# orhosko/tiny-ntt

Hardware: AMD Instinct MI355X
Metric: negacyclic poly-mults/sec (n=4096, 60-bit q), bit-exact vs cg_ntt.py (higher is better)
Workload: dtype u64; 1 GPU; n=4096, q=2^60-2^14+1 (60-bit), global batch 65536 = 65536 rows on this GPU, LCG-seeded rows resident in HBM (BASELINE configs[2]); n=4096, q=1152921504606830593, rows_per_gpu=65536, global_batch=65536, variant=fused, kernel=polymul_fused_kernel, lazy_reduction=True, lib_build_id=33db21926526ecac, parallelism=batch-sharded x1, no data-path collective

## Files before the change

tiny_ntt_amd/csrc/fused_core.h:

```cpp
#pragma once
#include <type_traits>
#include "modarith.h"

#ifndef TN_ABL_UNIFORM_TW
#define TN_ABL_UNIFORM_TW 0
#endif

namespace tn {

template <int B, int E_, typename F> struct StaticFor {
  TN_HD static void run(F& f) { f(std::integral_constant<int, B>()); StaticFor<B + 1, E_, F>::run(f); }
};
template <int E_, typename F> struct StaticFor<E_, E_, F> { TN_HD static void run(F&) {} };
template <int B, int E_, typename F> TN_HD void static_for(F&& f) { StaticFor<B, E_, F>::run(f); }

#ifndef TN_FUSED_LPT10
#define TN_FUSED_LPT10 3
#endif
#ifndef TN_FUSED_LPT12
#define TN_FUSED_LPT12 3
#endif
constexpr int fused_lpt(int logn) {
  return logn == 8 ? 2 : logn == 9 ? 3 : logn == 10 ? TN_FUSED_LPT10 : logn == 11 ? 3 : logn == 12 ? TN_FUSED_LPT12 : logn == 13 ? 3 : 0;
}

template <typename E> struct Arith {
  E q;
  u64 mu;
  int k;
  u32 fold_c;
  SplitK sk;
  u64 qmul[17];
  typename TwOf<E>::type one;
  typename TwOf<E>::type ninv;
  typename TwOf<E>::type fninv;
  typename TwOf<E>::type fninv_w1;
  typename TwOf<E>::type bninv;
  typename TwOf<E>::type bninv_w1;
};

template <typename E, int LOGN_, int LPT_> struct FusedCfg {
  static constexpr int LOGN = LOGN_, LPT = LPT_;
  static constexpr int N = 1 << LOGN, R = 1 << LPT, THREADS = N >> LPT;
  static constexpr int PHASES = (LOGN + LPT - 1) / LPT;
  static constexpr int pos(int p) { return (LOGN - (p + 1) * LPT) < 0 ? 0 : (LOGN - (p + 1) * LPT); }
  static constexpr int stage_begin(int p) { return p * LPT; }
  static constexpr int stage_end(int p) { return ((p + 1) * LPT) < LOGN ? ((p + 1) * LPT) : LOGN; }
  static constexpr int ex_pad(int e) { return pos(e + 1) > 0 ? (1 << pos(e + 1)) : 1; }
  static constexpr int ex_sh(int e) { return pos(e + 1) > 0 ? pos(e + 1) + LPT : LPT; }
  static constexpr int lay_span(int e, int cnt) { return cnt + ex_pad(e) * (cnt >> ex_sh(e)); }
  static constexpr int WB = (LOGN - LPT > 6) ? (LOGN - LPT - 6) : 0;
  static constexpr int WSH = LOGN - WB;
  static constexpr int tau_bit_to_j(int p, int t) { return t < pos(p) ? t : t + LPT; }
  static constexpr bool ex_wave_local(int e) {
    for (int t = 6; t < LOGN - LPT; ++t)
      if (tau_bit_to_j(e, t) != t + LPT || tau_bit_to_j(e + 1, t) != t + LPT) return false;
    return true;
  }
  static constexpr int region_elems() {
    int m = 1 << WSH;
    for (int e = 0; e + 1 < PHASES; ++e)
      if (ex_wave_local(e) && lay_span(e, 1 << WSH) > m) m = lay_span(e, 1 << WSH);
    return m;
  }
  static constexpr int lds_elems() {
    int m = region_elems() << WB;
    for (int e = 0; e + 1 < PHASES; ++e)
      if (!ex_wave_local(e) && lay_span(e, N) > m) m = lay_span(e, N);
    return m;
  }
  TN_HD static constexpr u32 jidx(int p, u32 tau, u32 r) {
    return ((tau >> pos(p)) << (pos(p) + LPT)) | (r << pos(p)) | (tau & ((1u << pos(p)) - 1u));
  }
  TN_HD static constexpr u32 ex_addr(int e, u32 j) {
    if (WB > 0 && ex_wave_local(e))
      return (j >> WSH) * (u32)region_elems() + (j & ((1u << WSH) - 1u)) + (u32)ex_pad(e) * ((j & ((1u << WSH) - 1u)) >> ex_sh(e));
    return j + (u32)ex_pad(e) * (j >> ex_sh(e));
  }
  TN_HD static constexpr u32 ex_base(int e, int p, u32 tau) { return ex_addr(e, jidx(p, tau, 0)); }
  TN_HD static constexpr u32 ex_off(int e, int p, u32 r) { return ex_addr(e, jidx(p, 0, r)); }
  enum { TW_UNIFORM = 0, TW_WAVE = 1, TW_LDS = 2, TW_REGS = 3, TW_VEC = 4 };
  static constexpr int LDS_TW_MAX_STAGE = 9;
  static constexpr int tw_src(int p) {
    return pos(p) >= LOGN - LPT ? TW_UNIFORM
         : (pos(p) >= 6 ? TW_WAVE : (pos(p) > 0 ? (stage_end(p) <= LDS_TW_MAX_STAGE ? TW_LDS : TW_VEC) : TW_REGS));
  }
  static constexpr int lds_tw_lo() {
    for (int p = 0; p < PHASES; ++p) if (tw_src(p) == TW_LDS) return 1 << stage_begin(p);
    return 0;
  }
  static constexpr int lds_tw_hi() {
    int h = 0;
    for (int p = 0; p < PHASES; ++p) if (tw_src(p) == TW_LDS) h = 1 << stage_end(p);
    return h;
  }
  static constexpr int lds_tw_count() { return lds_tw_hi() - lds_tw_lo(); }
  static constexpr int pre_count(int s) { return R >> ((LOGN - 1 - s) - pos(PHASES - 1) + 1); }
  static constexpr int pre_off(int s) {
    int o = 0;
    for (int i = stage_begin(PHASES - 1); i < s; ++i) o += pre_count(i);
    return o;
  }
  static constexpr int NPRE = (tw_src(PHASES - 1) == TW_REGS) ? pre_off(LOGN) : 1;
  TN_HD static u32 nat_addr(u32 k) { return k ^ ((k >> 5) & 15u); }
  TN_HD static u32 thi(int p, u32 tau) {
    if (pos(p) >= LOGN - LPT) return 0u;
    if (pos(p) >= 6) return wave_uniform(tau >> pos(p));
    return tau >> pos(p);
  }
};

template <typename E> struct LazyTraits;
template <> struct LazyTraits<u64> { static constexpr int LIMIT = 16, TMUL = 4, PW = 2; };
template <> struct LazyTraits<u32> { static constexpr int LIMIT = 64, TMUL = 2, PW = 4; };

template <typename E, bool LAZY, bool CIN = false> struct Policy {
  typedef typename TwOf<E>::type Tw;
  static constexpr bool lazy = LAZY;
  static constexpr bool canonical_inputs = CIN && LAZY && sizeof(E) == 8;
  static constexpr bool split = LAZY && sizeof(E) == 8;
  static constexpr int LIMIT = LazyTraits<E>::LIMIT, TMUL = LazyTraits<E>::TMUL, PW = LazyTraits<E>::PW;

  TN_HD static E load(E x, const Arith<E>& ar) {
    if (canonical_inputs) return x;
    if (LAZY) return fold(x, ar.k, ar.fold_c);
    return mul_tw(x, ar.one, ar.q);
  }
  TN_HD static E canon(E x, const Arith<E>& ar) {
    if (LAZY) { x = fold(x, ar.k, ar.fold_c); return csub(x, ar.q); }
    return x;
  }
  template <int K> TN_HD static void ct(E& u, E& v, Tw w, const Arith<E>& ar) {
    if constexpr (split) {
      const u64 x = mul_sp_acc(u, v, w, ar.sk);
      v = ((u << 1) + ar.qmul[K]) - x;
      u = x;
    } else if constexpr (LAZY) {
      const E t = mul_tw_lazy(v, w, ar.q);
      v = u + ((E)K * ar.q - t);
      u = u + t;
    } else {
      E t = mul_tw(v, w, ar.q);
      E s = u + t;
      v = u >= t ? u - t : u + (ar.q - t);
      u = csub(s, ar.q);
    }
  }
  template <int BND> TN_HD static void gs(E& u, E& v, Tw w, const Arith<E>& ar) {
    if constexpr (split) {
      const E d = (u + ar.qmul[BND]) - v;
      u = u + v;
      v = mul_sp(d, w, ar.sk);
    } else if constexpr (LAZY) {
      const E d = u + ((E)BND * ar.q - v);
      u = u + v;
      v = mul_tw_lazy(d, w, ar.q);
    } else {
      E d = u >= v ? u - v : u + (ar.q - v);
      u = csub(u + v, ar.q);
      v = mul_tw(d, w, ar.q);
    }
  }
  template <int BND> TN_HD static void gs_last(E& u, E& v, const Arith<E>& ar) {
    E d;
    if constexpr (split) d = (u + ar.qmul[BND]) - v;
    else d = LAZY ? (E)(u + ((E)BND * ar.q - v)) : (u >= v ? (E)(u - v) : (E)(u + (ar.q - v)));
    E s = u + v;
    u = mul_tw_canon(s, ar.fninv, ar);
    v = mul_tw_canon(d, ar.fninv_w1, ar);
  }
  TN_HD static E mul_tw_canon(E a, Tw w, const Arith<E>& ar) {
    if constexpr (split) return csub(fold(mul_sp(a, w, ar.sk), ar.k, ar.fold_c), ar.q);
    else return mul_tw(a, w, ar.q);
  }
};

template <typename P, int LOGN> struct Sched {
  static constexpr int fwd_in(int s) {
    int b = 2;
    for (int i = 0; i < s; ++i) { if (b + P::TMUL > P::LIMIT) b = 2; b += P::TMUL; }
    return b;
  }
  static constexpr bool fwd_fold(int s) { return P::lazy && fwd_in(s) + P::TMUL > P::LIMIT; }
  static constexpr int fwd_out() {
    int b = 2;
    for (int i = 0; i < LOGN; ++i) { if (b + P::TMUL > P::LIMIT) b = 2; b += P::TMUL; }
    return b;
  }
  static constexpr int inv_in(int g) {
    int b = P::lazy ? P::PW : 1;
    for (int i = 0; i < g; ++i) { if (2 * b > P::LIMIT) b = 2; b = (2 * b > P::TMUL) ? 2 * b : P::TMUL; }
    return b;
  }
  static constexpr bool inv_fold(int g) { return P::lazy && 2 * inv_in(g) > P::LIMIT; }
  static constexpr int inv_bnd(int g) { return inv_fold(g) ? 2 : inv_in(g); }
};

template <typename Cfg, bool CIN = false, bool BC = false> struct SplitSched {
  static constexpr int LOGN = Cfg::LOGN, R = Cfg::R;
  static constexpr int FEND = BC ? LOGN - 1 : LOGN;
  static constexpr long U = 4096, CAP = 16 * U;
  static constexpr long FOLDED = U + 1;
  static constexpr long PW_OUT = 2 * U;
  static constexpr long PW_IN = 14 * (U - 1);
  static constexpr long tmax(long bv) { return 4 * U + (bv + 7) / 8 + 2; }
  static constexpr long BC_AMAX = CAP - 8;
  static constexpr int kq(long b) { return (int)((b + U - 2) / (U - 1)); }
  static constexpr int kf(long t) { return kq(t) <= 6 ? 6 : kq(t); }
  static constexpr int ki(long b) { return (kq(b) + 3) / 4 * 4; }
  static constexpr int phase_of(int s) { return s / Cfg::LPT; }
  static constexpr int bpos_of(int s) { return (LOGN - 1 - s) - Cfg::pos(phase_of(s)); }
  struct Data {
    bool ffold[LOGN][R] = {};
    unsigned char fk[LOGN][R] = {};
    long fout = 0;
    bool pw_fold_b = false;
    bool bcfold[R] = {};
    bool ifold[LOGN][R] = {};
    unsigned char ik[LOGN][R] = {};
  };
  static constexpr Data build() {
    Data d;
    long b[R] = {};
    for (int r = 0; r < R; ++r) b[r] = CIN ? U : (r < R / 2 ? FOLDED : CAP);
    for (int s = 0; s < FEND; ++s) {
      if (s > 0 && phase_of(s) != phase_of(s - 1)) {
        long m = 0;
        for (int r = 0; r < R; ++r) m = b[r] > m ? b[r] : m;
        for (int r = 0; r < R; ++r) b[r] = m;
      }
// ... 255 lines not shown
```

tiny_ntt_amd/csrc/kernels.hip:

```cpp
#include <hip/hip_runtime.h>
#include "plan.h"
#include "dev_addr.h"

#ifndef TN_ABL_NO_BARRIER
#define TN_ABL_NO_BARRIER 0
#endif
#ifndef TN_ABL_ROWMASK
#define TN_ABL_ROWMASK 0
#endif
#ifndef TN_ABL_NO_GLOBAL
#define TN_ABL_NO_GLOBAL 0
#endif
#ifndef TN_STORE_AT_TOP
#define TN_STORE_AT_TOP 1
#endif
#ifndef TN_NT_STREAM
#define TN_NT_STREAM 1
#endif
#ifndef TN_FUSED_MIN_WAVES
#define TN_FUSED_MIN_WAVES 4
#endif
#ifndef TN_POLYMUL60_WAVES
#define TN_POLYMUL60_WAVES 6
#endif

#ifndef TN_NTTF_PIN_LOGN
#define TN_NTTF_PIN_LOGN 99
#endif
#ifndef TN_VEC_PREFETCH
#define TN_VEC_PREFETCH 1
#endif
#ifndef TN_FUSED_CIN
#define TN_FUSED_CIN 0
#endif
#ifndef TN_SADDR
#define TN_SADDR 1
#endif
#ifndef TN_KARG_ARITH
#define TN_KARG_ARITH 1
#endif
#ifndef TN_RESIDENT_TW
#define TN_RESIDENT_TW 1
#endif
#ifndef TN_SHARE_MID_TW
#define TN_SHARE_MID_TW 1
#endif
#ifndef TN_SHARE_LAST_TW
#define TN_SHARE_LAST_TW 1
#endif
#ifdef TN_MARKS
#define TN_MARK(n) asm volatile("; TNMARK " n)
#else
#define TN_MARK(n)
#endif
namespace tn {

#ifndef TN_SHUFFLE_LAST
#define TN_SHUFFLE_LAST 0
#endif
template <int DIST> __device__ __forceinline__ u32 lane_xor(u32 v) {
  if constexpr (DIST == 1) return (u32)__builtin_amdgcn_update_dpp(0, (int)v, 0xB1, 0xf, 0xf, false);
  else if constexpr (DIST == 2) return (u32)__builtin_amdgcn_update_dpp(0, (int)v, 0x4E, 0xf, 0xf, false);
  else {
    int r = __builtin_amdgcn_update_dpp(0, (int)v, 0x104, 0xf, 0x5, false);
    return (u32)__builtin_amdgcn_update_dpp(r, (int)v, 0x114, 0xf, 0xA, false);
  }
}
template <typename E>
__device__ __forceinline__ void transpose8_lanes(E (&x)[8], u32 lane) {
  static_for<0, 3>([&](auto b_) {
    constexpr int b = decltype(b_)::value, m = 1 << b;
    const bool hi = (lane >> b) & 1u;
    static_for<0, 8>([&](auto r_) {
      constexpr int r0 = decltype(r_)::value;
      if constexpr (!(r0 & m)) {
        constexpr int r1 = r0 | m;
        const E send = hi ? x[r0] : x[r1];
        E recv;
        if constexpr (sizeof(E) == 8) recv = ((u64)lane_xor<m>((u32)(send >> 32)) << 32) | lane_xor<m>((u32)send);
        else recv = lane_xor<m>((u32)send);
        x[r0] = hi ? recv : x[r0];
        x[r1] = hi ? x[r1] : recv;
      }
    });
  });
}

template <typename E, typename Cfg, int EX, int FROM, int TO>
__device__ __forceinline__ void exchange(E (&x)[Cfg::R], u32 tau, E* lds) {
  if constexpr (TN_SHUFFLE_LAST && Cfg::LPT == 3 && EX == Cfg::PHASES - 2 && Cfg::pos(EX + 1) == 0 && Cfg::pos(EX) == Cfg::LPT) {
    transpose8_lanes<E>(x, tau);
  } else if constexpr (Cfg::ex_wave_local(EX)) {
    __builtin_amdgcn_wave_barrier();
    ex_store<E, Cfg, EX, FROM>(x, tau, lds);
    __builtin_amdgcn_wave_barrier();
    ex_load<E, Cfg, EX, TO>(x, tau, lds);
    __builtin_amdgcn_wave_barrier();
  } else {
#if TN_ABL_NO_BARRIER
    __builtin_amdgcn_wave_barrier();
    ex_store<E, Cfg, EX, FROM>(x, tau, lds);
    __builtin_amdgcn_wave_barrier();
    ex_load<E, Cfg, EX, TO>(x, tau, lds);
    __builtin_amdgcn_wave_barrier();
#else
    __syncthreads();
    ex_store<E, Cfg, EX, FROM>(x, tau, lds);
    __syncthreads();
    ex_load<E, Cfg, EX, TO>(x, tau, lds);
    __syncthreads();
#endif
  }
}

template <typename E>
__device__ __forceinline__ const Arith<E>& kernarg_arith(u32 zero) {
  typedef const __attribute__((address_space(4))) char* KP;
  return *(const Arith<E>*)((KP)__builtin_amdgcn_kernarg_segment_ptr() + zero);
}

template <typename E, typename Cfg, typename Pol, int P0, int P1, bool KARG = false, int PRE_END = Cfg::LOGN, bool BC = false>
__device__ __forceinline__ void forward_range(E (&x)[Cfg::R], u32 tau, const TwRefs<E>& tw_in, const Arith<E>& ar_in, E* lds, bool fetch_pre,
                                              u32 tau_g) {
  typename TwOf<E>::type vec[Cfg::R];
  static_for<P0, P1>([&](auto p_) {
    constexpr int p = decltype(p_)::value;
    constexpr bool FULL = Cfg::stage_end(p) - Cfg::stage_begin(p) == Cfg::LPT;
    TN_MARK("fwd_phase");
    TwRefs<E> tw = tw_in;
    if constexpr (KARG) tw.zero = opaque_zero();
    if constexpr (TN_VEC_PREFETCH && Cfg::tw_src(p) == Cfg::TW_VEC && FULL && p > P0) tw.mid = vec;
    const Arith<E>& ar = KARG ? kernarg_arith<E>(tw.zero) : ar_in;
    fwd_phase<E, Cfg, Pol, p, BC>(x, tau, tw, ar);
    TN_MARK("fwd_other");
    if constexpr (p == Cfg::PHASES - 2) {
      if (fetch_pre) {
        sched_fence();
        tw_prefetch_stages<E, Cfg, Cfg::stage_begin(Cfg::PHASES - 1), PRE_END>(tw.pre, tau_g, tw.glob);
        sched_fence();
      }
    }
    if constexpr (p + 1 < P1) {
      constexpr int pn = p + 1 < Cfg::PHASES ? p + 1 : p;
      if constexpr (TN_VEC_PREFETCH && Cfg::tw_src(pn) == Cfg::TW_VEC && Cfg::stage_end(pn) - Cfg::stage_begin(pn) == Cfg::LPT) {
        sched_fence();
        tw_fetch_vec<E, Cfg, pn>(vec, tau_g, tw.glob);
        sched_fence();
      }
    }
    if constexpr (p + 1 < Cfg::PHASES) exchange<E, Cfg, p, p, p + 1>(x, tau, lds);
  });
}
template <typename E, typename Cfg, typename Pol>
__device__ __forceinline__ void forward_all(E (&x)[Cfg::R], u32 tau, const typename TwOf<E>::type* __restrict__ glob,
                                            const typename TwOf<E>::type* lds_tw, const Arith<E>& ar, E* lds, u32 zero = 0) {
  typename TwOf<E>::type pre[Cfg::NPRE];
  const TwRefs<E> tw = {glob, lds_tw, pre, nullptr, zero};
  forward_range<E, Cfg, Pol, 0, Cfg::PHASES>(x, tau, tw, ar, lds, true, tau);
}

template <typename E, typename Cfg, typename Pol, bool KARG = false, bool BC = false, typename F>
__device__ __forceinline__ void inverse_all(E (&x)[Cfg::R], u32 tau, const TwRefs<E>& tw_in, const Arith<E>& ar_in, E* lds,
                                            F&& after_first) {
  typename TwOf<E>::type vec[Cfg::R];
  static_for<0, Cfg::PHASES>([&](auto i_) {
    constexpr int p = Cfg::PHASES - 1 - decltype(i_)::value;
    constexpr bool FULL = Cfg::stage_end(p) - Cfg::stage_begin(p) == Cfg::LPT;
    TN_MARK("inv_phase");
    TwRefs<E> tw = tw_in;
    if constexpr (KARG) tw.zero = opaque_zero();
    if constexpr (TN_VEC_PREFETCH && Cfg::tw_src(p) == Cfg::TW_VEC && FULL && p < Cfg::PHASES - 1) tw.mid = vec;
    const Arith<E>& ar = KARG ? kernarg_arith<E>(tw.zero) : ar_in;
    inv_phase<E, Cfg, Pol, p, BC>(x, tau, tw, ar);
    TN_MARK("inv_other");
    if constexpr (p > 0) {
      constexpr int pn = p > 0 ? p - 1 : 0;
      if constexpr (TN_VEC_PREFETCH && Cfg::tw_src(pn) == Cfg::TW_VEC && Cfg::stage_end(pn) - Cfg::stage_begin(pn) == Cfg::LPT) {
        sched_fence();
        tw_fetch_vec<E, Cfg, pn>(vec, tau, tw.glob);
        sched_fence();
      }
    }
    if constexpr (p == Cfg::PHASES - 1) { sched_fence(); after_first(); sched_fence(); }
    if constexpr (p > 0) exchange<E, Cfg, p - 1, p, p - 1>(x, tau, lds);
  });
}

template <typename E> struct alignas(2 * sizeof(E)) PairOf { E lo, hi; };

#ifdef TN_FUSED_STAMPS
__device__ unsigned long long tn_fused_stamps[4 * 4096];
#endif

template <typename E, typename Cfg>
__device__ __forceinline__ E ld_operand(const E* __restrict__ p, u32 row, u32 tau, int r) {
#if TN_ABL_NO_GLOBAL
  return (E)(tau * 2654435761u + 7 * r + row);
#else
#if TN_ABL_ROWMASK
  row &= TN_ABL_ROWMASK;
#endif
#if TN_NT_STREAM
  const TN_GLOBAL_AS E* rp = uniform_ptr(p + ((size_t)row << Cfg::LOGN) + Cfg::jidx(0, 0, r));
  return __builtin_nontemporal_load(rp + (Cfg::jidx(0, tau, 0) & (u32)(Cfg::N - 1)));
#else
  return p[((size_t)row << Cfg::LOGN) + Cfg::jidx(0, tau, r)];
#endif
#endif
}

template <typename E, typename Cfg>
__device__ __forceinline__ void st_result(E* __restrict__ c, u32 row, u32 tau, const E (&x)[Cfg::R]) {
#if TN_ABL_ROWMASK
  row &= TN_ABL_ROWMASK;
#endif
  const size_t off = (size_t)row << Cfg::LOGN;
#pragma unroll
  for (int r = 0; r < Cfg::R; ++r) {
#if TN_NT_STREAM
    __builtin_nontemporal_store(x[r], uniform_ptr(c + off + Cfg::jidx(0, 0, r)) + (Cfg::jidx(0, tau, 0) & (u32)(Cfg::N - 1)));
#else
    c[off + Cfg::jidx(0, tau, r)] = x[r];
#endif
  }
}

template <typename E, int LOGN, int LPT, bool LAZY>
constexpr int polymul_waves() {
  return LPT >= 4 ? 2 : (sizeof(E) == 8 && LOGN == 12 && LAZY) ? TN_POLYMUL60_WAVES : TN_FUSED_MIN_WAVES;
}

template <typename E, int LOGN, int LPT, bool LAZY, bool CIN = false, bool BC = false>
__global__ void __launch_bounds__((1 << (LOGN - LPT)), (polymul_waves<E, LOGN, LPT, LAZY>()))
polymul_fused_kernel(const Arith<E> ar, const typename TwOf<E>::type* __restrict__ tab_fwd,
                     const typename TwOf<E>::type* __restrict__ tab_inv, const E* __restrict__ a, const E* __restrict__ b,
                     E* __restrict__ c, u32 batch, u32* sched, u32 chunk) {
  typedef FusedCfg<E, LOGN, LPT> Cfg;
  typedef Policy<E, LAZY, CIN> Pol;
  extern __shared__ __attribute__((aligned(16))) unsigned char tn_smem[];
  E* lds = reinterpret_cast<E*>(tn_smem);
  typedef typename TwOf<E>::type Tw;
  const u32 tau = threadIdx.x;
  Tw* lds_fwd = reinterpret_cast<Tw*>(lds + Cfg::lds_elems());
  Tw* lds_inv = lds_fwd + Cfg::lds_tw_count();
  u32* lds_next = reinterpret_cast<u32*>(lds_inv + Cfg::lds_tw_count());
  for (u32 i = tau; i < (u32)Cfg::lds_tw_count(); i += Cfg::THREADS) {
    lds_fwd[i] = tab_fwd[Cfg::lds_tw_lo() + i];
    lds_inv[i] = tab_inv[Cfg::lds_tw_lo() + i];
  }
  __syncthreads();
  E xa[Cfg::R], xb[Cfg::R];
#ifdef TN_FUSED_STAMPS
  const unsigned long long st_t0 = __builtin_amdgcn_s_memtime(), st_r0 = __builtin_amdgcn_s_memrealtime();
#endif
  u32 row = blockIdx.x * chunk;
  u32 taken = 1;
  u32 chunk_id = blockIdx.x;
  if (row < batch) {
#pragma unroll
    for (int r = 0; r < Cfg::R; ++r) xb[r] = ld_operand<E, Cfg>(a, row, tau, r);
  }
  constexpr int PRE_END = (TN_RESIDENT_TW && polymul_waves<E, LOGN, LPT, LAZY>() <= 4 && Cfg::stage_end(Cfg::PHASES - 1) - Cfg::stage_begin(Cfg::PHASES - 1) >= 2) ? Cfg::LOGN - 1 : Cfg::LOGN;
  Tw prf[Cfg::NPRE];
  tw_prefetch_stages<E, Cfg, PRE_END, Cfg::LOGN>(prf, tau, tab_fwd);
  u32 prev = row;
  bool have_c = false;
#pragma unroll
  for (int r = 0; r < Cfg::R; ++r) xa[r] = 0;
  while (row < batch) {
    const u32 zero = opaque_zero();
    const u32 tl = opaque_copy(tau);
    const bool in_chunk = taken != chunk;
    taken = in_chunk ? taken + 1 : 1;
    chunk_id = in_chunk ? chunk_id : chunk_id + gridDim.x;
    if (tau == 0) *lds_next = in_chunk ? row + 1 : (sched ? gridDim.x + atomicAdd(&sched[0], 1u) : chunk_id) * chunk;
    TN_MARK("loop_top");
    E xn[Cfg::R];
#pragma unroll
    for (int r = 0; r < Cfg::R; ++r) xn[r] = xb[r];
    load_reduce<E, Cfg, Pol>(xn, ar);
    sched_fence();
#if TN_STORE_AT_TOP
    st_result<E, Cfg>(c, prev, tl, xa);
#endif
#pragma unroll
    for (int r = 0; r < Cfg::R; ++r) xb[r] = ld_operand<E, Cfg>(b, row, tl, r);
    sched_fence();
#pragma unroll
    for (int r = 0; r < Cfg::R; ++r) xa[r] = xn[r];
    constexpr bool KARG = TN_KARG_ARITH != 0;
    constexpr bool SHARE = TN_SHARE_LAST_TW && Cfg::PHASES >= 2;
    constexpr int PM = Cfg::PHASES >= 3 ? Cfg::PHASES - 2 : 0;
    constexpr bool SHARE2 = SHARE && TN_SHARE_MID_TW && Cfg::PHASES >= 3 && Cfg::tw_src(PM) == Cfg::TW_LDS &&
                            Cfg::stage_end(PM) - Cfg::stage_begin(PM) == Cfg::LPT;
    const TwRefs<E> twf = {tab_fwd, lds_fwd, prf, nullptr, zero};
    static_assert(!BC || SHARE2, "base case: built for the shared-twiddle schedule only");
    if constexpr (SHARE2) forward_range<E, Cfg, Pol, 0, PM, KARG, Cfg::LOGN, BC>(xa, tau, twf, ar, lds, false, tl);
    else if constexpr (SHARE) forward_range<E, Cfg, Pol, 0, Cfg::PHASES - 1, KARG>(xa, tau, twf, ar, lds, false, tl);
    else forward_all<E, Cfg, Pol>(xa, tau, tab_fwd, lds_fwd, ar, lds, zero);
    __syncthreads();
    const u32 next = wave_uniform(*lds_next);
    load_reduce<E, Cfg, Pol>(xb, ar);
    if constexpr (SHARE2) {
      forward_range<E, Cfg, Pol, 0, PM, KARG, Cfg::LOGN, BC>(xb, tau, twf, ar, lds, false, tl);
      Tw mid[Cfg::R];
      tw_fetch_mid<E, Cfg, PM>(mid, tau, lds_fwd);
      const TwRefs<E> twm = {tab_fwd, lds_fwd, prf, mid, zero};
      forward_range<E, Cfg, Pol, PM, PM + 1, KARG, Cfg::LOGN, BC>(xa, tau, twm, ar, lds, false, tl);
      forward_range<E, Cfg, Pol, PM, PM + 1, KARG, PRE_END, BC>(xb, tau, twm, ar, lds, true, tl);
      forward_range<E, Cfg, Pol, PM + 1, Cfg::PHASES, KARG, Cfg::LOGN, BC>(xb, tau, twf, ar, lds, false, tl);
      forward_range<E, Cfg, Pol, PM + 1, Cfg::PHASES, KARG, Cfg::LOGN, BC>(xa, tau, twf, ar, lds, false, tl);
    } else if constexpr (SHARE) {
      forward_range<E, Cfg, Pol, 0, Cfg::PHASES - 1, KARG, PRE_END>(xb, tau, twf, ar, lds, true, tl);
      forward_range<E, Cfg, Pol, Cfg::PHASES - 1, Cfg::PHASES, KARG>(xb, tau, twf, ar, lds, false, tl);
      forward_range<E, Cfg, Pol, Cfg::PHASES - 1, Cfg::PHASES, KARG>(xa, tau, twf, ar, lds, false, tl);
    } else {
      forward_all<E, Cfg, Pol>(xb, tau, tab_fwd, lds_fwd, ar, lds, zero);
    }
    Tw pre[Cfg::NPRE];
    if constexpr (BC) {
      TN_MARK("basecase");
      basecase<Cfg, Pol>(xa, xb, prf + Cfg::pre_off(Cfg::LOGN - 1), ar);
      sched_fence();
      tw_prefetch_stages<E, Cfg, Cfg::stage_begin(Cfg::PHASES - 1), Cfg::LOGN - 1>(pre, tl, tab_inv);
    } else {
      tw_prefetch<E, Cfg>(pre, tl, tab_inv);
      TN_MARK("pointwise");
      pointwise<E, Cfg, Pol>(xa, xb, ar);
    }
    TN_MARK("after_pointwise");
    const TwRefs<E> twi = {tab_inv, lds_inv, pre, nullptr, zero};
    inverse_all<E, Cfg, Pol, KARG, BC>(xa, tau, twi, ar, lds, [&]() {
      const u32 nrow = next < batch ? next : row;
#pragma unroll
      for (int r = 0; r < Cfg::R; ++r) xb[r] = ld_operand<E, Cfg>(a, nrow, tl, r);
    });
#if TN_STORE_AT_TOP
    prev = row;
    have_c = true;
#else
    st_result<E, Cfg>(c, row, tau, xa);
#endif
    row = next;
  }
  if (have_c) st_result<E, Cfg>(c, prev, tau, xa);
#ifdef TN_FUSED_STAMPS
  if (tau == 0 && blockIdx.x < 4096) {
    tn_fused_stamps[4 * blockIdx.x + 0] = st_t0; tn_fused_stamps[4 * blockIdx.x + 1] = st_r0;
    tn_fused_stamps[4 * blockIdx.x + 2] = __builtin_amdgcn_s_memtime(); tn_fused_stamps[4 * blockIdx.x + 3] = __builtin_amdgcn_s_memrealtime();
  }
#endif
  if (sched && tau == 0 && atomicAdd(&sched[1], 1u) == gridDim.x - 1) { sched[0] = 0; sched[1] = 0; }
}

template <typename E, int LOGN, int LPT, bool LAZY, int MODE>
__global__ void __launch_bounds__((1 << (LOGN - LPT)), (LPT >= 4 ? 2 : TN_FUSED_MIN_WAVES))
ntt_fused_kernel(const Arith<E> ar, const typename TwOf<E>::type* __restrict__ tab, const E* __restrict__ in, E* __restrict__ out, u32 batch,
                 u32* sched, u32 chunk) {
  typedef FusedCfg<E, LOGN, LPT> Cfg;
  typedef Policy<E, LAZY> Pol;
  typedef typename TwOf<E>::type Tw;
  extern __shared__ __attribute__((aligned(16))) unsigned char tn_smem[];
  E* lds = reinterpret_cast<E*>(tn_smem);
  const u32 tau = threadIdx.x;
  E* nat = lds + Cfg::lds_elems();
  Tw* lds_tab = reinterpret_cast<Tw*>(nat + Cfg::N);
  u32* lds_next = reinterpret_cast<u32*>(lds_tab + Cfg::lds_tw_count());
  for (u32 i = tau; i < (u32)Cfg::lds_tw_count(); i += Cfg::THREADS) lds_tab[i] = tab[Cfg::lds_tw_lo() + i];
  u32 left = chunk - 1, chunk_id = blockIdx.x;
  auto take_next = [&](u32 cur, u32 slot) {
    if (left) { --left; lds_next[slot] = cur + 1; }
    else {
      chunk_id = sched ? gridDim.x + atomicAdd(&sched[0], 1u) : chunk_id + gridDim.x;
      left = chunk - 1;
      lds_next[slot] = chunk_id * chunk;
    }
  };
  if (tau == 0) take_next(blockIdx.x * chunk, 1u);
  __syncthreads();
  u32 next = wave_uniform(lds_next[1]);
  constexpr int LAST = Cfg::PHASES - 1;
  E xn[Cfg::R];
  u32 row = blockIdx.x * chunk;
  if (row < batch) {
#pragma unroll
    for (int r = 0; r < Cfg::R; ++r) xn[r] = ld_operand<E, Cfg>(in, row, tau, r);
  }
  for (u32 it = 0; row < batch; ++it) {
    if (tau == 0) take_next(next, it & 1u);
    constexpr bool PIN = LOGN >= TN_NTTF_PIN_LOGN;
    const u32 zero = PIN ? opaque_zero() : 0u;
    const u32 tl = PIN ? opaque_copy(tau) : tau;
    constexpr bool KARG = PIN && TN_KARG_ARITH != 0;
    E x[Cfg::R];
#pragma unroll
    for (int r = 0; r < Cfg::R; ++r) x[r] = xn[r];
    sched_fence();
    if (MODE != FNTT_CYCLIC_INV && next < batch) {
#pragma unroll
      for (int r = 0; r < Cfg::R; ++r) xn[r] = ld_operand<E, Cfg>(in, next, tl, r);
    }
    sched_fence();
    if (MODE == FNTT_CYCLIC_INV) {
#pragma unroll
      for (int r = 0; r < Cfg::R; ++r) x[r] = Pol::load(x[r], ar);
#pragma unroll
      for (int r = 0; r < Cfg::R; ++r) nat[Cfg::nat_addr(Cfg::jidx(0, tau, r))] = x[r];
      __syncthreads();
#pragma unroll
      for (int r = 0; r < Cfg::R; ++r) x[r] = nat[Cfg::nat_addr(bitrev(Cfg::jidx(LAST, tau, r), LOGN))];
      Tw pre[Cfg::NPRE];
      tw_prefetch<E, Cfg>(pre, tl, tab);
      const TwRefs<E> tw = {tab, lds_tab, pre, nullptr, zero};
      inverse_all<E, Cfg, Pol, KARG>(x, tau, tw, ar, lds, [&]() {
        if (next < batch) {
#pragma unroll
          for (int r = 0; r < Cfg::R; ++r) xn[r] = ld_operand<E, Cfg>(in, next, tl, r);
        }
      });
      st_result<E, Cfg>(out, row, tl, x);
    } else {
#pragma unroll
      for (int r = 0; r < Cfg::R / 2; ++r) x[r] = Pol::load(x[r], ar);
      if (!LAZY) {
#pragma unroll
        for (int r = Cfg::R / 2; r < Cfg::R; ++r) x[r] = Pol::load(x[r], ar);
      }
      {
        Tw pre[Cfg::NPRE];
        const TwRefs<E> tw = {tab, lds_tab, pre, nullptr, zero};
        forward_range<E, Cfg, Pol, 0, Cfg::PHASES, KARG>(x, tau, tw, ar, lds, true, tl);
      }
#pragma unroll
      for (int r = 0; r < Cfg::R; ++r)
        nat[Cfg::nat_addr(bitrev(Cfg::jidx(LAST, tau, r), LOGN))] = LAZY ? Pol::canon(x[r], ar) : x[r];
      __syncthreads();
#pragma unroll
      for (int r = 0; r < Cfg::R; ++r) x[r] = nat[Cfg::nat_addr(Cfg::jidx(0, tau, r))];
      st_result<E, Cfg>(out, row, tl, x);
    }
    if (Cfg::THREADS <= 64) __syncthreads();
    row = next;
    next = wave_uniform(lds_next[it & 1u]);
  }
  if (sched && tau == 0 && atomicAdd(&sched[1], 1u) == gridDim.x - 1) { sched[0] = 0; sched[1] = 0; }
}

template <typename E, int LOGN, int LPT, bool LAZY>
static hipError_t launch_nttf_t(const tn_plan* p, int mode, const void* in, void* out, size_t batch, hipStream_t s) {
  typedef FusedCfg<E, LOGN, LPT> Cfg;
  typedef typename TwOf<E>::type Tw;
  const size_t lds_bytes = (size_t)(Cfg::lds_elems() + Cfg::N) * sizeof(E) + (size_t)Cfg::lds_tw_count() * sizeof(Tw) + 16;
  const PlanView<E> pv = make_view<E>(p);
  auto kern = ntt_fused_kernel<E, LOGN, LPT, LAZY, FNTT_TWIST_FWD>;
  if (mode == FNTT_CYCLIC_FWD) kern = ntt_fused_kernel<E, LOGN, LPT, LAZY, FNTT_CYCLIC_FWD>;
  else if (mode != FNTT_TWIST_FWD) kern = ntt_fused_kernel<E, LOGN, LPT, LAZY, FNTT_CYCLIC_INV>;
  const FusedNttSetup<E> su = fused_ntt_setup(pv.ar, mode);
  return launch_persistent(p, s, (const void*)kern, Cfg::THREADS, lds_bytes, Cfg::N * sizeof(E), batch, FUSED_ROWS, [&](u32 grid, u32* sched, u32 chunk) {
    const Tw* tab = fused_table(pv, su.tab);
    const E* in_ = (const E*)in; E* out_ = (E*)out; u32 b32 = (u32)batch;
    Arith<E> ar = su.ar;
    void* args[] = {&ar, &tab, &in_, &out_, &b32, &sched, &chunk};
    return hipLaunchKernel((const void*)kern, dim3(grid), dim3(Cfg::THREADS), args, lds_bytes, s);
  });
}

template <typename E, bool LAZY>
static hipError_t launch_nttf_e(const tn_plan* p, int mode, const void* in, void* out, size_t batch, hipStream_t s) {
#ifdef TN_ONLY_MAIN
  return hipErrorInvalidValue;
#else
  switch (p->logn) {
    case 8: return launch_nttf_t<E, 8, fused_lpt(8), LAZY>(p, mode, in, out, batch, s);
    case 9: return launch_nttf_t<E, 9, fused_lpt(9), LAZY>(p, mode, in, out, batch, s);
    case 10: return launch_nttf_t<E, 10, fused_lpt(10), LAZY>(p, mode, in, out, batch, s);
    case 11: return launch_nttf_t<E, 11, fused_lpt(11), LAZY>(p, mode, in, out, batch, s);
    case 12: return launch_nttf_t<E, 12, fused_lpt(12), LAZY>(p, mode, in, out, batch, s);
    case 13: return launch_nttf_t<E, 13, fused_lpt(13), LAZY>(p, mode, in, out, batch, s);
    default: return hipErrorInvalidValue;
  }
#endif
}

hipError_t launch_ntt_fused(const tn_plan* p, int mode, const void* in, void* out, size_t batch, hipStream_t s) {
  if (batch == 0) return hipSuccess;
  if (p->elem_bytes == 8)
    return p->lazy ? launch_nttf_e<u64, true>(p, mode, in, out, batch, s) : launch_nttf_e<u64, false>(p, mode, in, out, batch, s);
  return p->lazy ? launch_nttf_e<u32, true>(p, mode, in, out, batch, s) : launch_nttf_e<u32, false>(p, mode, in, out, batch, s);
}

bool fused_supported(u32 logn, int) { return fused_lpt((int)logn) != 0; }

template <typename E, int LOGN, int LPT, bool LAZY>
static hipError_t launch_fused_t(const tn_plan* p, const void* a, const void* b, void* c, size_t batch, hipStream_t s, bool cyclic) {
  typedef FusedCfg<E, LOGN, LPT> Cfg;
  const size_t lds_bytes = (size_t)Cfg::lds_elems() * sizeof(E) +
                           (size_t)2 * Cfg::lds_tw_count() * sizeof(typename TwOf<E>::type) + 16;
  constexpr bool HAS_CIN = TN_FUSED_CIN && sizeof(E) == 8 && LOGN == 12 && LAZY;
  constexpr bool HAS_BC = fused_has_bc<E, LOGN, LPT, LAZY>();
  const bool use_cin = HAS_CIN && p->canonical_inputs && !cyclic;
  const bool use_bc = HAS_BC && p->bc_ok && !use_cin;
  auto kern = polymul_fused_kernel<E, LOGN, LPT, LAZY>;
// ... 211 lines not shown
```

tiny_ntt_amd/csrc/launch_plan.h:

```cpp
#pragma once
#include <stddef.h>
#include "fused_core.h"

#ifndef TN_DYNAMIC_ROWS
#define TN_DYNAMIC_ROWS 1
#endif
#ifndef TN_SCHED_CHUNK_BYTES
#define TN_SCHED_CHUNK_BYTES 32768
#endif
#ifndef TN_CG_DYNAMIC_ROWS
#define TN_CG_DYNAMIC_ROWS 1
#endif
#ifndef TN_CG_DYNAMIC_MIN
#define TN_CG_DYNAMIC_MIN 8
#endif
#ifndef TN_CG_CHUNK_BYTES
#define TN_CG_CHUNK_BYTES 32768
#endif

namespace tn {

enum FusedNttMode { FNTT_TWIST_FWD = 0, FNTT_CYCLIC_FWD = 1, FNTT_CYCLIC_INV = 2 };

enum FusedTable { FT_PSI_BRV, FT_PSI_INV_BRV, FT_CYC_BRV, FT_CYC_INV_BRV, FT_PSI_BC, FT_CYC_BC };

constexpr int FUSED_BC_LOGN = 12;
template <typename E, int LOGN, int LPT, bool LAZY> constexpr bool fused_has_bc() {
  return sizeof(E) == 8 && LOGN == FUSED_BC_LOGN && LPT == 3 && LAZY;
}

template <typename E> struct FusedProductSetup { bool bc; Arith<E> ar; FusedTable fwd, inv; };
template <typename E> inline FusedProductSetup<E> fused_product_setup(const Arith<E>& ar, bool bc, bool cyclic) {
  FusedProductSetup<E> s = {bc, ar, cyclic ? FT_CYC_BRV : FT_PSI_BRV, cyclic ? FT_CYC_INV_BRV : FT_PSI_INV_BRV};
  if (bc) { s.ar.fninv = ar.bninv; s.ar.fninv_w1 = ar.bninv_w1; s.fwd = cyclic ? FT_CYC_BC : FT_PSI_BC; }
  if (cyclic) s.ar.fninv_w1 = s.ar.fninv;
  return s;
}

template <typename E> struct FusedNttSetup { Arith<E> ar; FusedTable tab; };
template <typename E> inline FusedNttSetup<E> fused_ntt_setup(const Arith<E>& ar, int mode) {
  FusedNttSetup<E> s = {ar, mode == FNTT_TWIST_FWD ? FT_PSI_BRV : mode == FNTT_CYCLIC_FWD ? FT_CYC_BRV : FT_CYC_INV_BRV};
  if (mode == FNTT_CYCLIC_INV) s.ar.fninv_w1 = s.ar.fninv;
  return s;
}

struct RowPolicy { size_t chunk_bytes, min_chunks; bool enabled, single_rows_without_slot; };
constexpr RowPolicy FUSED_ROWS = {TN_SCHED_CHUNK_BYTES, 4, TN_DYNAMIC_ROWS != 0, false};
constexpr RowPolicy CG_ROWS = {TN_CG_CHUNK_BYTES, TN_CG_DYNAMIC_MIN, TN_CG_DYNAMIC_ROWS != 0, true};

struct RowPlan { u32 chunk; bool dynamic; };
inline RowPlan plan_rows(size_t row_bytes, size_t batch, size_t resident, const RowPolicy& pol) {
  size_t want = pol.chunk_bytes / row_bytes;
  if (want < 1) want = 1;
  if (pol.enabled && batch >= pol.min_chunks * resident * want) return {(u32)want, true};
  return {1u, false};
}

}
```

Baseline: 30.55 million poly-mults/s.

## Drop redundant workgroup barriers around cross-wave LDS exchanges in fused polymul

Makes the leading and trailing __syncthreads around each cross-wave LDS transpose configurable. In the base-case path it replaces them with wave barriers wherever a constexpr ownership analysis shows each wave only touches its own LDS region on that side. It also removes the mid-row barrier that published the next row index, reading it later instead. This cuts workgroup-wide synchronisation stalls per row, at the risk of LDS races if the ownership reasoning is wrong. Optional region-timing instrumentation is added but compiled out by default.

```diff
diff --git a/tiny_ntt_amd/csrc/fused_core.h b/tiny_ntt_amd/csrc/fused_core.h
--- a/tiny_ntt_amd/csrc/fused_core.h
+++ b/tiny_ntt_amd/csrc/fused_core.h
@@ -76,6 +76,12 @@
     if (WB > 0 && ex_wave_local(e))
       return (j >> WSH) * (u32)region_elems() + (j & ((1u << WSH) - 1u)) + (u32)ex_pad(e) * ((j & ((1u << WSH) - 1u)) >> ex_sh(e));
     return j + (u32)ex_pad(e) * (j >> ex_sh(e));
+  }
+  static constexpr bool ex_side_wave_own(int e, int p) {
+    for (u32 tau = 0; tau < (u32)THREADS; ++tau)
+      for (u32 r = 0; r < (u32)R; ++r)
+        if (ex_addr(e, jidx(p, tau, r)) / (u32)region_elems() != (tau >> 6)) return false;
+    return true;
   }
   TN_HD static constexpr u32 ex_base(int e, int p, u32 tau) { return ex_addr(e, jidx(p, tau, 0)); }
   TN_HD static constexpr u32 ex_off(int e, int p, u32 r) { return ex_addr(e, jidx(p, 0, r)); }
diff --git a/tiny_ntt_amd/csrc/kernels.hip b/tiny_ntt_amd/csrc/kernels.hip
--- a/tiny_ntt_amd/csrc/kernels.hip
+++ b/tiny_ntt_amd/csrc/kernels.hip
@@ -45,6 +45,9 @@
 #ifndef TN_SHARE_MID_TW
 #define TN_SHARE_MID_TW 1
 #endif
+#ifndef TN_LEAN_BARRIERS
+#define TN_LEAN_BARRIERS 15
+#endif
 #ifndef TN_SHARE_LAST_TW
 #define TN_SHARE_LAST_TW 1
 #endif
@@ -54,6 +57,32 @@
 #define TN_MARK(n)
 #endif
 namespace tn {
+
+#ifdef TN_FUSED_STAMPS
+enum { RGN_A = 0, RGN_B = 16, RGN_INV = 32,
+       RGN_LOOP_TOP = 48, RGN_MID = 49, RGN_B_LOAD = 50, RGN_BASECASE = 51, RGN_AFTER_FIRST = 52, RGN_ROW = 62, RGN_ROWS = 63, RGN_COUNT = 64 };
+__device__ __forceinline__ unsigned long long* rgn_acc() {
+  __shared__ unsigned long long acc[RGN_COUNT];
+  return acc;
+}
+template <int ID, bool END> __device__ __forceinline__ void rgn_stamp() {
+  if constexpr (ID >= 0) {
+    sched_fence();
+    if (threadIdx.x == 0) {
+      const unsigned long long t = __builtin_amdgcn_s_memtime();
+      __hip_atomic_fetch_add(rgn_acc() + ID, END ? t : 0ull - t, __ATOMIC_RELAXED, __HIP_MEMORY_SCOPE_WORKGROUP);
+    }
+    sched_fence();
+  }
+}
+#define TN_RGN_BEGIN(id) rgn_stamp<(id), false>()
+#define TN_RGN_END(id) rgn_stamp<(id), true>()
+#define TN_RGN(base, off) ((base) < 0 ? -1 : (base) + (off))
+#else
+#define TN_RGN_BEGIN(id)
+#define TN_RGN_END(id)
+#define TN_RGN(base, off) (-1)
+#endif
 
 #ifndef TN_SHUFFLE_LAST
 #define TN_SHUFFLE_LAST 0
@@ -86,7 +115,7 @@
   });
 }
 
-template <typename E, typename Cfg, int EX, int FROM, int TO>
+template <typename E, typename Cfg, int EX, int FROM, int TO, int XBAR = XBAR_ALL, int RGW = -1>
 __device__ __forceinline__ void exchange(E (&x)[Cfg::R], u32 tau, E* lds) {
   if constexpr (TN_SHUFFLE_LAST && Cfg::LPT == 3 && EX == Cfg::PHASES - 2 && Cfg::pos(EX + 1) == 0 && Cfg::pos(EX) == Cfg::LPT) {
     transpose8_lanes<E>(x, tau);
@@ -104,11 +133,17 @@
     ex_load<E, Cfg, EX, TO>(x, tau, lds);
     __builtin_amdgcn_wave_barrier();
 #else
+    TN_RGN_BEGIN(RGW);
+    if constexpr (XBAR & XBAR_LEAD) __syncthreads(); else __builtin_amdgcn_wave_barrier();
+    TN_RGN_END(RGW);
+    ex_store<E, Cfg, EX, FROM>(x, tau, lds);
+    TN_RGN_BEGIN(RGW);
     __syncthreads();
-    ex_store<E, Cfg, EX, FROM>(x, tau, lds);
-    __syncthreads();
+    TN_RGN_END(RGW);
     ex_load<E, Cfg, EX, TO>(x, tau, lds);
-    __syncthreads();
+    TN_RGN_BEGIN(RGW);
+    if constexpr (XBAR & XBAR_TRAIL) __syncthreads(); else __builtin_amdgcn_wave_barrier();
+    TN_RGN_END(RGW);
 #endif
   }
 }
@@ -119,7 +154,8 @@
   return *(const Arith<E>*)((KP)__builtin_amdgcn_kernarg_segment_ptr() + zero);
 }
 
-template <typename E, typename Cfg, typename Pol, int P0, int P1, bool KARG = false, int PRE_END = Cfg::LOGN, bool BC = false>
+template <typename E, typename Cfg, typename Pol, int P0, int P1, bool KARG = false, int PRE_END = Cfg::LOGN, bool BC = false, int XBAR = XBAR_ALL,
+          int RG = -1>
 __device__ __forceinline__ void forward_range(E (&x)[Cfg::R], u32 tau, const TwRefs<E>& tw_in, const Arith<E>& ar_in, E* lds, bool fetch_pre,
                                               u32 tau_g) {
   typename TwOf<E>::type vec[Cfg::R];
@@ -127,6 +163,7 @@
     constexpr int p = decltype(p_)::value;
     constexpr bool FULL = Cfg::stage_end(p) - Cfg::stage_begin(p) == Cfg::LPT;
     TN_MARK("fwd_phase");
+    TN_RGN_BEGIN(TN_RGN(RG, 4 * p));
     TwRefs<E> tw = tw_in;
     if constexpr (KARG) tw.zero = opaque_zero();
     if constexpr (TN_VEC_PREFETCH && Cfg::tw_src(p) == Cfg::TW_VEC && FULL && p > P0) tw.mid = vec;
@@ -148,7 +185,12 @@
         sched_fence();
       }
     }
-    if constexpr (p + 1 < Cfg::PHASES) exchange<E, Cfg, p, p, p + 1>(x, tau, lds);
+    TN_RGN_END(TN_RGN(RG, 4 * p));
+    if constexpr (p + 1 < Cfg::PHASES) {
+      TN_RGN_BEGIN(TN_RGN(RG, 4 * p + 1));
+      exchange<E, Cfg, p, p, p + 1, XBAR, TN_RGN(RG, 4 * p + 2)>(x, tau, lds);
+      TN_RGN_END(TN_RGN(RG, 4 * p + 1));
+    }
   });
 }
 template <typename E, typename Cfg, typename Pol>
@@ -159,7 +201,7 @@
   forward_range<E, Cfg, Pol, 0, Cfg::PHASES>(x, tau, tw, ar, lds, true, tau);
 }
 
-template <typename E, typename Cfg, typename Pol, bool KARG = false, bool BC = false, typename F>
+template <typename E, typename Cfg, typename Pol, bool KARG = false, bool BC = false, int XBAR = XBAR_ALL, int RG = -1, typename F>
 __device__ __forceinline__ void inverse_all(E (&x)[Cfg::R], u32 tau, const TwRefs<E>& tw_in, const Arith<E>& ar_in, E* lds,
                                             F&& after_first) {
   typename TwOf<E>::type vec[Cfg::R];
@@ -167,6 +209,7 @@
     constexpr int p = Cfg::PHASES - 1 - decltype(i_)::value;
     constexpr bool FULL = Cfg::stage_end(p) - Cfg::stage_begin(p) == Cfg::LPT;
     TN_MARK("inv_phase");
+    TN_RGN_BEGIN(TN_RGN(RG, 4 * p));
     TwRefs<E> tw = tw_in;
     if constexpr (KARG) tw.zero = opaque_zero();
     if constexpr (TN_VEC_PREFETCH && Cfg::tw_src(p) == Cfg::TW_VEC && FULL && p < Cfg::PHASES - 1) tw.mid = vec;
@@ -181,15 +224,20 @@
         sched_fence();
       }
     }
+    TN_RGN_END(TN_RGN(RG, 4 * p));
     if constexpr (p == Cfg::PHASES - 1) { sched_fence(); after_first(); sched_fence(); }
-    if constexpr (p > 0) exchange<E, Cfg, p - 1, p, p - 1>(x, tau, lds);
+    if constexpr (p > 0) {
+      TN_RGN_BEGIN(TN_RGN(RG, 4 * p - 3));
+      exchange<E, Cfg, p - 1, p, p - 1, XBAR, TN_RGN(RG, 4 * p - 2)>(x, tau, lds);
+      TN_RGN_END(TN_RGN(RG, 4 * p - 3));
+    }
   });
 }
 
 template <typename E> struct alignas(2 * sizeof(E)) PairOf { E lo, hi; };
 
 #ifdef TN_FUSED_STAMPS
-__device__ unsigned long long tn_fused_stamps[4 * 4096];
+__device__ unsigned long long tn_fused_stamps[(4 + 64) * 4096];
 #endif
 
 template <typename E, typename Cfg>
@@ -252,6 +300,11 @@
   E xa[Cfg::R], xb[Cfg::R];
 #ifdef TN_FUSED_STAMPS
   const unsigned long long st_t0 = __builtin_amdgcn_s_memtime(), st_r0 = __builtin_amdgcn_s_memrealtime();
+  if (tau < RGN_COUNT) rgn_acc()[tau] = 0;
+  __syncthreads();
+  constexpr int RGA = RGN_A, RGB = RGN_B, RGI = RGN_INV;
+#else
+  constexpr int RGA = -1, RGB = -1, RGI = -1;
 #endif
   u32 row = blockIdx.x * chunk;
   u32 taken = 1;
@@ -268,6 +321,8 @@
 #pragma unroll
   for (int r = 0; r < Cfg::R; ++r) xa[r] = 0;
   while (row < batch) {
+    TN_RGN_BEGIN(RGN_ROW);
+    TN_RGN_BEGIN(RGN_LOOP_TOP);
     const u32 zero = opaque_zero();
     const u32 tl = opaque_copy(tau);
     const bool in_chunk = taken != chunk;
@@ -288,6 +343,7 @@
     sched_fence();
 #pragma unroll
     for (int r = 0; r < Cfg::R; ++r) xa[r] = xn[r];
+    TN_RGN_END(RGN_LOOP_TOP);
     constexpr bool KARG = TN_KARG_ARITH != 0;
     constexpr bool SHARE = TN_SHARE_LAST_TW && Cfg::PHASES >= 2;
     constexpr int PM = Cfg::PHASES >= 3 ? Cfg::PHASES - 2 : 0;
@@ -295,21 +351,32 @@
                             Cfg::stage_end(PM) - Cfg::stage_begin(PM) == Cfg::LPT;
     const TwRefs<E> twf = {tab_fwd, lds_fwd, prf, nullptr, zero};
     static_assert(!BC || SHARE2, "base case: built for the shared-twiddle schedule only");
-    if constexpr (SHARE2) forward_range<E, Cfg, Pol, 0, PM, KARG, Cfg::LOGN, BC>(xa, tau, twf, ar, lds, false, tl);
+    constexpr int LEAN = BC && fused_lean_barriers<Cfg>() ? TN_LEAN_BARRIERS : 0;
+    static_assert(!BC || LEAN == TN_LEAN_BARRIERS, "base case: the lean barrier placement needs transpose 0's phase-1 side wave-own");
+    constexpr int XA = fused_xbar_a(LEAN), XF = fused_xbar_fwd(LEAN), XI = fused_xbar_inv(LEAN);
+    if constexpr (SHARE2) forward_range<E, Cfg, Pol, 0, PM, KARG, Cfg::LOGN, BC, XA, RGA>(xa, tau, twf, ar, lds, false, tl);
     else if constexpr (SHARE) forward_range<E, Cfg, Pol, 0, Cfg::PHASES - 1, KARG>(xa, tau, twf, ar, lds, false, tl);
     else forward_all<E, Cfg, Pol>(xa, tau, tab_fwd, lds_fwd, ar, lds, zero);
-    __syncthreads();
-    const u32 next = wave_uniform(*lds_next);
+    u32 next = 0;
+    if constexpr (!(LEAN & LEAN_NO_MID)) {
+      TN_RGN_BEGIN(RGN_MID);
+      __syncthreads();
+      next = wave_uniform(*lds_next);
+      TN_RGN_END(RGN_MID);
+    }
+    TN_RGN_BEGIN(RGN_B_LOAD);
     load_reduce<E, Cfg, Pol>(xb, ar);
+    TN_RGN_END(RGN_B_LOAD);
     if constexpr (SHARE2) {
-      forward_range<E, Cfg, Pol, 0, PM, KARG, Cfg::LOGN, BC>(xb, tau, twf, ar, lds, false, tl);
+      forward_range<E, Cfg, Pol, 0, PM, KARG, Cfg::LOGN, BC, XF, RGB>(xb, tau, twf, ar, lds, false, tl);
+      if constexpr (LEAN & LEAN_NO_MID) next = wave_uniform(*lds_next);
       Tw mid[Cfg::R];
       tw_fetch_mid<E, Cfg, PM>(mid, tau, lds_fwd);
       const TwRefs<E> twm = {tab_fwd, lds_fwd, prf, mid, zero};
-      forward_range<E, Cfg, Pol, PM, PM + 1, KARG, Cfg::LOGN, BC>(xa, tau, twm, ar, lds, false, tl);
-      forward_range<E, Cfg, Pol, PM, PM + 1, KARG, PRE_END, BC>(xb, tau, twm, ar, lds, true, tl);
-      forward_range<E, Cfg, Pol, PM + 1, Cfg::PHASES, KARG, Cfg::LOGN, BC>(xb, tau, twf, ar, lds, false, tl);
-      forward_range<E, Cfg, Pol, PM + 1, Cfg::PHASES, KARG, Cfg::LOGN, BC>(xa, tau, twf, ar, lds, false, tl);
+      forward_range<E, Cfg, Pol, PM, PM + 1, KARG, Cfg::LOGN, BC, XF, RGA>(xa, tau, twm, ar, lds, false, tl);
+      forward_range<E, Cfg, Pol, PM, PM + 1, KARG, PRE_END, BC, XF, RGB>(xb, tau, twm, ar, lds, true, tl);
+      forward_range<E, Cfg, Pol, PM + 1, Cfg::PHASES, KARG, Cfg::LOGN, BC, XF, RGB>(xb, tau, twf, ar, lds, false, tl);
+      forward_range<E, Cfg, Pol, PM + 1, Cfg::PHASES, KARG, Cfg::LOGN, BC, XF, RGA>(xa, tau, twf, ar, lds, false, tl);
     } else if constexpr (SHARE) {
       forward_range<E, Cfg, Pol, 0, Cfg::PHASES - 1, KARG, PRE_END>(xb, tau, twf, ar, lds, true, tl);
       forward_range<E, Cfg, Pol, Cfg::PHASES - 1, Cfg::PHASES, KARG>(xb, tau, twf, ar, lds, false, tl);
@@ -320,9 +387,11 @@
     Tw pre[Cfg::NPRE];
     if constexpr (BC) {
       TN_MARK("basecase");
+      TN_RGN_BEGIN(RGN_BASECASE);
       basecase<Cfg, Pol>(xa, xb, prf + Cfg::pre_off(Cfg::LOGN - 1), ar);
       sched_fence();
       tw_prefetch_stages<E, Cfg, Cfg::stage_begin(Cfg::PHASES - 1), Cfg::LOGN - 1>(pre, tl, tab_inv);
+      TN_RGN_END(RGN_BASECASE);
     } else {
       tw_prefetch<E, Cfg>(pre, tl, tab_inv);
       TN_MARK("pointwise");
@@ -330,11 +399,17 @@
     }
     TN_MARK("after_pointwise");
     const TwRefs<E> twi = {tab_inv, lds_inv, pre, nullptr, zero};
-    inverse_all<E, Cfg, Pol, KARG, BC>(xa, tau, twi, ar, lds, [&]() {
+    inverse_all<E, Cfg, Pol, KARG, BC, XI, RGI>(xa, tau, twi, ar, lds, [&]() {
+      TN_RGN_BEGIN(RGN_AFTER_FIRST);
       const u32 nrow = next < batch ? next : row;
 #pragma unroll
       for (int r = 0; r < Cfg::R; ++r) xb[r] = ld_operand<E, Cfg>(a, nrow, tl, r);
+      TN_RGN_END(RGN_AFTER_FIRST);
     });
+    TN_RGN_END(RGN_ROW);
+#ifdef TN_FUSED_STAMPS
+    if (tau == 0) __hip_atomic_fetch_add(rgn_acc() + RGN_ROWS, 1ull, __ATOMIC_RELAXED, __HIP_MEMORY_SCOPE_WORKGROUP);
+#endif
 #if TN_STORE_AT_TOP
     prev = row;
     have_c = true;
@@ -348,6 +423,7 @@
   if (tau == 0 && blockIdx.x < 4096) {
     tn_fused_stamps[4 * blockIdx.x + 0] = st_t0; tn_fused_stamps[4 * blockIdx.x + 1] = st_r0;
     tn_fused_stamps[4 * blockIdx.x + 2] = __builtin_amdgcn_s_memtime(); tn_fused_stamps[4 * blockIdx.x + 3] = __builtin_amdgcn_s_memrealtime();
+    for (int i = 0; i < RGN_COUNT; ++i) tn_fused_stamps[4 * 4096 + RGN_COUNT * blockIdx.x + i] = rgn_acc()[i];
   }
 #endif
   if (sched && tau == 0 && atomicAdd(&sched[1], 1u) == gridDim.x - 1) { sched[0] = 0; sched[1] = 0; }
diff --git a/tiny_ntt_amd/csrc/launch_plan.h b/tiny_ntt_amd/csrc/launch_plan.h
--- a/tiny_ntt_amd/csrc/launch_plan.h
+++ b/tiny_ntt_amd/csrc/launch_plan.h
@@ -29,6 +29,46 @@
   return sizeof(E) == 8 && LOGN == FUSED_BC_LOGN && LPT == 3 && LAZY;
 }
 
+enum { XBAR_LEAD = 1, XBAR_MID = 2, XBAR_TRAIL = 4, XBAR_ALL = 7 };
+
+enum { LEAN_NO_MID = 1, LEAN_INV_TRAIL = 2, LEAN_OWN_SIDE = 4, LEAN_A_LEAD = 8, LEAN_ALL = 15 };
+constexpr int fused_xbar_fwd(int lean) { return (lean & LEAN_OWN_SIDE) ? XBAR_LEAD | XBAR_MID : XBAR_ALL; }
+constexpr int fused_xbar_a(int lean) { return fused_xbar_fwd(lean) & ~((lean & LEAN_A_LEAD) ? XBAR_LEAD : 0); }
+constexpr int fused_xbar_inv(int lean) {
+  return XBAR_MID | ((lean & LEAN_OWN_SIDE) ? 0 : XBAR_LEAD) | ((lean & LEAN_INV_TRAIL) ? 0 : XBAR_TRAIL);
+}
+template <typename Cfg> constexpr bool fused_lean_barriers() {
+  if (Cfg::PHASES < 3 || Cfg::ex_wave_local(0) || !Cfg::ex_side_wave_own(0, 1)) return false;
+  for (int e = 1; e + 1 < Cfg::PHASES; ++e) if (!Cfg::ex_wave_local(e)) return false;
+  return true;
+}
+
+struct LdsStep { char op; int ex, phase, use; };
+template <typename Cfg, typename Emit>
+inline void fused_product_lds_steps(int lean, Emit&& emit) {
+  const int xa = fused_xbar_a(lean), xfwd = fused_xbar_fwd(lean), xinv = fused_xbar_inv(lean);
+  const bool mid_barrier = !(lean & LEAN_NO_MID);
+  int use = 0;
+  auto transpose = [&](int ex, int from, int to, int xbar) {
+    const bool cross = !Cfg::ex_wave_local(ex);
+    if (cross && (xbar & XBAR_LEAD)) emit(LdsStep{'B', 0, 0, 0});
+    emit(LdsStep{'S', ex, from, use});
+    if (cross) emit(LdsStep{'B', 0, 0, 0});
+    emit(LdsStep{'L', ex, to, use});
+    if (cross && (xbar & XBAR_TRAIL)) emit(LdsStep{'B', 0, 0, 0});
+    ++use;
+  };
+  constexpr int PM = Cfg::PHASES - 2;
+  emit(LdsStep{'W', 0, 0, 0});
+  for (int p = 0; p < PM; ++p) transpose(p, p, p + 1, xa);
+  if (mid_barrier) { emit(LdsStep{'B', 0, 0, 0}); emit(LdsStep{'R', 0, 0, 0}); }
+  for (int p = 0; p < PM; ++p) transpose(p, p, p + 1, xfwd);
+  if (!mid_barrier) emit(LdsStep{'R', 0, 0, 0});
+  transpose(PM, PM, PM + 1, xfwd);
+  transpose(PM, PM, PM + 1, xfwd);
+  for (int p = Cfg::PHASES - 1; p > 0; --p) transpose(p - 1, p, p - 1, xinv);
+}
+
 template <typename E> struct FusedProductSetup { bool bc; Arith<E> ar; FusedTable fwd, inv; };
 template <typename E> inline FusedProductSetup<E> fused_product_setup(const Arith<E>& ar, bool bc, bool cyclic) {
   FusedProductSetup<E> s = {bc, ar, cyclic ? FT_CYC_BRV : FT_PSI_BRV, cyclic ? FT_CYC_INV_BRV : FT_PSI_INV_BRV};
```

Measured after the change: 30.80 million poly-mults/s (median of 6 runs). No clear change (+0.8%).
